# alexpreynolds/starch3

Hardware: AMD Instinct MI355X
Metric: input BED MB/s (cfg2, bzip2 -9, archive bit-identical to CPU starch3 path) (higher is better)
Workload: dtype u8

## Files before the change

### starch_amd/csrc/bz2_bwt3.hip

```cpp
#include "bz2_int.hpp"
#include "bz2_bwt.hpp"

#include <algorithm>
#include <type_traits>

namespace bz {
namespace {

constexpr int PT = 256;
constexpr int PTILE = 32768;
constexpr int PDIG = 12;
constexpr int PNB = 1 << PDIG;
constexpr int PNB_WIDE = 8192;
static_assert(PTILE <= 32768 && PNB_WIDE <= 8192, "k3_scatter_lds packs (digit << 15) | rotation-in-tile");
constexpr int MAXT = (900064 + PTILE - 1) / PTILE;
constexpr uint32_t W_MAX = 64, S1_MAX = 128, S_MAX = 256, M0_MAX = 512, M1_MAX = 1024, M2_MAX = 2048, M3_MAX = 4096;
#ifndef STARCH_L_MIN
#define STARCH_L_MIN 4096
#endif
constexpr uint32_t L_MIN = STARCH_L_MIN;
constexpr uint32_t GB_MIN = 16384;
constexpr uint32_t GB_MAXN = 8192;
constexpr uint32_t HG_MIN_PUSH = 32768;
constexpr uint32_t RBITS = 20;
// ... 1451 lines not shown
            const uint64_t item = shfl64(myitem, gi);
            const uint32_t goff = (uint32_t)__shfl((int)off, (int)gi, 64);
            const uint32_t gstart = valid ? goff : 0u;
            const uint32_t slot = it_slot(item), s = it_start(item), m = it_size(item), par = it_par(item);
            const uint32_t j = valid ? lane - gstart : 0u;
            const uint32_t* sv = (par ? c.scr.V : c.scr.SA) + (uint64_t)slot * c.scr.stride + s;
            const KeySrc ks = key_src(c, slot, par);
            const uint32_t v = sv[j];
            uint32_t ls;
            uint64_t k = elem_key<DBL>(c, ks, slot, s + j, v, ls);
            if (!valid) k = ~0ull;
            uint32_t r = 0;
            if (ng == 1) {
                for (uint32_t q = 0; q < total; ++q) {
                    const uint64_t kq = ((uint64_t)(uint32_t)__builtin_amdgcn_readlane((int)(k >> 32), (int)q) << 32) |
                                        (uint32_t)__builtin_amdgcn_readlane((int)(uint32_t)k, (int)q);
                    r += (kq < k || (kq == k && q < j)) ? 1u : 0u;
                }
            } else {
                const uint32_t maxm = wave_reduce_max(valid ? m : 0u);
                for (uint32_t q = 0; q < maxm; ++q) {
                    const bool in = valid && q < m;
                    const uint64_t kq = shfl64(k, in ? gstart + q : lane);
                    r += (in && (kq < k || (kq == k && q < j))) ? 1u : 0u;
                }
            }
            wave_sync_lds3();
            if (valid) { skey[wid][gstart + r] = k; sval[wid][gstart + r] = v | (ls << 24); }
            wave_sync_lds3();
            const uint64_t key = valid ? skey[wid][lane] : 0;
            const uint32_t val = valid ? sval[wid][lane] : 0;
            const bool head = valid && (j == 0 || skey[wid][lane - 1] != key);
            const bool end = valid && (j + 1 == m || skey[wid][lane + 1] != key);
            const uint32_t hp = wave_incl_scan_max<uint32_t>(head ? lane : 0u) - gstart;
            asm volatile("s_waitcnt vmcnt(0)" ::: "memory");
            uint32_t runs = 0;
            emit_sorted(c, slot, s, j, val & 0xFFFFFFu, valid, hp, end, runs, val >> 24);
            if (c.mode) {
                const uint64_t em = __ballot(end);
                const uint64_t gm = (m >= 64 ? ~0ull : ((1ull << m) - 1ull)) << gstart;
                wave_add_slot(c.L.runs, valid && j == 0, slot, (uint32_t)__popcll(em & gm));
            }
            done += ng;
        }
    }
}

#ifndef STARCH_RANK_UNROLL
#define STARCH_RANK_UNROLL 4
#endif
__device__ __forceinline__ uint32_t rank_in(const uint64_t* xk, uint32_t rs, uint32_t re, uint64_t kj)
{
    uint32_t r = 0;
    uint32_t q = rs;
    if constexpr (STARCH_RANK_UNROLL >= 8) {
        for (; q + 8 <= re; q += 8) {
            uint64_t x[8];
#pragma unroll
            for (int i = 0; i < 8; ++i) x[i] = xk[q + i];
#pragma unroll
            for (int i = 0; i < 8; ++i) r += x[i] < kj ? 1u : 0u;
        }
    }
    if constexpr (STARCH_RANK_UNROLL != 0) {
        for (; q + 4 <= re; q += 4) {
            const uint64_t a = xk[q], b = xk[q + 1], c2 = xk[q + 2], d = xk[q + 3];
            r += (a < kj ? 1u : 0u) + (b < kj ? 1u : 0u) + (c2 < kj ? 1u : 0u) + (d < kj ? 1u : 0u);
        }
    }
    for (; q < re; ++q) r += xk[q] < kj ? 1u : 0u;
    return r;
}

template <int NW>
__device__ __forceinline__ void gsync()
{
    if constexpr (NW == 1) wave_sync_lds3();
    else __syncthreads();
}

template <int E>
struct GrpIn {
    uint64_t item;
    KeySrc ks;
    uint32_t v[E];
    uint32_t v0;
    uint64_t kx[E];
    uint32_t ls[E];
    uint64_t k0;
    uint64_t kb[E];
    uint32_t lb[E];
    uint64_t k0b;
    bool one;
};

template <int NW, int E>
__device__ __forceinline__ void grp_load_vals(const Ctx& c, GrpIn<E>& x, bool ok, int wid, int lane)
{
    if (!ok) x.item = mk_item(0, 0, 1, 0, 0);
    const uint32_t slot = it_slot(x.item), s = it_start(x.item), m = it_size(x.item), par = it_par(x.item);
    const uint32_t* sv = (par ? c.scr.V : c.scr.SA) + (uint64_t)slot * c.scr.stride + s;
    x.ks = key_src(c, slot, par);
#pragma unroll
    for (int e = 0; e < E; ++e) {
        const uint32_t i = (uint32_t)(wid * 64 * E + e * 64 + lane);
        x.v[e] = sv[i < m ? i : 0u];
    }
    x.v0 = sv[0];
}

__device__ __forceinline__ uint32_t pss_rr(const KeySrc& ks, uint32_t r)
{
    const uint32_t rr = r + ks.off;
    return rr >= ks.n ? rr - ks.n : rr;
}
__device__ __forceinline__ uint32_t pss_pr(const KeySrc& ks, uint32_t r) { return r ? r - 1u : ks.n - 1u; }

template <int NW, bool DBL>
constexpr bool defer_keys() { return !DBL && NW == 1; }

template <int NW, int E, bool DBL>
__device__ __forceinline__ void grp_load_keys(const Ctx& c, GrpIn<E>& x, int wid, int lane)
{
    const uint32_t s = it_start(x.item), m = it_size(x.item), slot = it_slot(x.item);
    if constexpr (!defer_keys<NW, DBL>()) {
#pragma unroll
        for (int e = 0; e < E; ++e) {
            const uint32_t i = (uint32_t)(wid * 64 * E + e * 64 + lane);
            x.kx[e] = elem_key<DBL>(c, x.ks, slot, s + (i < m ? i : 0u), x.v[e], x.ls[e]);
        }
        x.k0 = elem_key<DBL>(x.ks, s, x.v0);
    } else {
        const uint64_t* __restrict__ w = x.ks.pss;
        const uint32_t* __restrict__ w32 = reinterpret_cast<const uint32_t*>(w);
        const uint32_t B = x.ks.B;
        x.one = x.ks.off == 0 && (B == 1 || B == 2 || B == 4 || B == 5 || B == 6 || B == 8);
        if (x.one) {
#pragma unroll
            for (int e = 0; e < E; ++e) {
                const uint32_t r = x.v[e];
                const uint64_t q = ((uint64_t)(r ? r - 1u : 0u) * B) >> 6;
                const uint4 kv = *reinterpret_cast<const uint4*>(w + q);
                x.kx[e] = ((uint64_t)kv.y << 32) | kv.x;
                x.kb[e] = ((uint64_t)kv.w << 32) | kv.z;
                if (r == 0) {
                    const uint64_t j = ((uint64_t)(x.ks.n - 1u) * B) >> 5;
                    x.ls[e] = w32[j ^ 1u];
                    x.lb[e] = w32[(j + 1u) ^ 1u];
                }
            }
        } else {
#pragma unroll
            for (int e = 0; e < E; ++e) {
                const uint64_t q = ((uint64_t)pss_rr(x.ks, x.v[e]) * B) >> 6;
                x.kx[e] = w[q];
                x.kb[e] = w[q + 1];
                const uint64_t j = ((uint64_t)pss_pr(x.ks, x.v[e]) * B) >> 5;
                x.ls[e] = w32[j ^ 1u];
                x.lb[e] = w32[(j + 1u) ^ 1u];
            }
        }
        const uint64_t q0 = ((uint64_t)pss_rr(x.ks, x.v0) * x.ks.B) >> 6;
        x.k0 = w[q0];
        x.k0b = w[q0 + 1];
    }
}

template <int NW, int E, bool DBL>
__device__ __forceinline__ void grp_finish_keys(GrpIn<E>& x)
{
    if constexpr (defer_keys<NW, DBL>()) {
        const KeySrc& ks = x.ks;
        if (x.one) {
            const uint32_t B = ks.B;
#pragma unroll
            for (int e = 0; e < E; ++e) {
                const uint32_t r = x.v[e];
                const uint64_t A = x.kx[e], W = x.kb[e];
                if (r) {
                    const uint32_t p0 = (uint32_t)(((uint64_t)(r - 1u) * B) & 63u), pk = p0 + B;
                    x.ls[e] = (uint32_t)(((A << p0) | ((W >> 1) >> (63u - p0))) >> (64u - B));
                    const uint64_t win = pk >= 64u ? (W << (pk - 64u)) : ((A << pk) | ((W >> 1) >> (63u - pk)));
                    x.kx[e] = win >> (64u - ks.kbits);
                } else {
                    x.kx[e] = A >> (64u - ks.kbits);
                    const uint32_t pl = (uint32_t)(((uint64_t)(ks.n - 1u) * B) & 31u);
                    const uint64_t lw = ((uint64_t)x.ls[e] << 32) | x.lb[e];
                    x.ls[e] = (uint32_t)((lw << pl) >> (64u - B));
                }
            }
        } else {
#pragma unroll
        for (int e = 0; e < E; ++e) {
            const uint32_t p = (uint32_t)(((uint64_t)pss_rr(ks, x.v[e]) * ks.B) & 63u);
            const uint64_t v = (x.kx[e] << p) | ((x.kb[e] >> 1) >> (63u - p));
            x.kx[e] = v >> (64u - ks.kbits);
            const uint32_t pl = (uint32_t)(((uint64_t)pss_pr(ks, x.v[e]) * ks.B) & 31u);
            const uint64_t lw = ((uint64_t)x.ls[e] << 32) | x.lb[e];
            x.ls[e] = (uint32_t)((lw << pl) >> (64u - ks.B));
        }
        }
        const uint32_t p0 = (uint32_t)(((uint64_t)pss_rr(ks, x.v0) * ks.B) & 63u);
        const uint64_t v0 = (x.k0 << p0) | ((x.k0b >> 1) >> (63u - p0));
        x.k0 = v0 >> (64u - ks.kbits);
    }
}

#ifndef STARCH_WPE_GRP
#define STARCH_WPE_GRP 1
#endif
#ifndef STARCH_WPE_M2
#define STARCH_WPE_M2 3
#endif
#ifndef STARCH_WPE_S
#define STARCH_WPE_S STARCH_WPE_GRP
#endif
#ifndef STARCH_WPE_M1
#define STARCH_WPE_M1 1
#endif
#ifndef STARCH_WPE_M0
#define STARCH_WPE_M0 6
#endif
constexpr int sort_wpe(int NW, int E)
{
    return NW == 4 && E == 8   ? STARCH_WPE_M2
           : NW == 4 && E == 4 ? STARCH_WPE_M1
           : NW == 4 && E == 2 ? STARCH_WPE_M0
           : (NW == 1 ? (E == 2 ? STARCH_WPE_S : STARCH_WPE_GRP) : 1);
}

template <int NW, int E, bool DBL>
__global__ void __launch_bounds__(NW > 4 ? 64 * NW : 256) __attribute__((amdgpu_waves_per_eu(sort_wpe(NW, E))))
k3_sort_lds(Ctx c, const uint64_t* __restrict__ items,
                                                    const uint32_t* __restrict__ hard_n)
{
    constexpr int IPW = NW >= 4 ? 1 : 4 / NW;
    constexpr int NWV = IPW * NW;
    constexpr int CAP = NW * 64 * E;
    constexpr int IDXB = CAP <= 256 ? 8 : 12;
    constexpr int KEYB = 64 - IDXB;
    constexpr uint64_t KMASK = (1ull << KEYB) - 1ull;
    constexpr int DPT = NW >= 4 ? 1 : 256 / (64 * NW);
    static_assert(CAP <= (1 << IDXB), "index does not fit");
#ifndef STARCH_M2_DB
#define STARCH_M2_DB 11
#endif
    constexpr int DB = CAP <= 128 ? 7 : (CAP <= 256 ? 8 : (CAP <= 1024 ? 10 : (CAP == 2048 ? STARCH_M2_DB : 11)));
    constexpr int NBIN = 1 << DB;
    constexpr int T = NW * 64;
    constexpr int BPT = NBIN / T;
#ifndef STARCH_LIM_NUM
#define STARCH_LIM_NUM 256
#endif
#ifndef STARCH_LIM2_NUM
#define STARCH_LIM2_NUM 512
#endif
    constexpr uint32_t LIMIT = STARCH_LIM_NUM / E;
    __shared__ uint64_t xk_all[IPW][CAP];
    __shared__ uint32_t vb_all[IPW][CAP];
    __shared__ uint16_t bst_all[IPW][NBIN + 2];
    constexpr int UR = NBIN > 256 * NW ? NBIN : 256 * NW;
    __shared__ uint32_t ur_all[IPW][UR];
    __shared__ uint32_t sc_all[IPW][NW + 1];
    constexpr int NB2 = NW == 1 ? 256 : 1024;
    constexpr uint32_t LIMIT2 = STARCH_LIM2_NUM / E;
    __shared__ uint32_t c2_all[IPW][NB2 + 1];
    __shared__ uint32_t sc2_all[IPW][NW + 1];
    __shared__ uint64_t red_all[NWV];
    __shared__ uint32_t wmax_all[NWV];
    __shared__ uint32_t flag_all[NWV];
    __shared__ uint32_t tc_all[NW + 1 > 5 ? NW + 1 : 5];
    uint32_t tacc = 0;
    const int tid = threadIdx.x, lane = tid & 63, wave = tid >> 6;
    const int g = wave / NW, wid = wave % NW, w0 = g * NW;
    uint64_t* xk = xk_all[g];
    uint32_t* wcnt = ur_all[g] + wid * 256;
    uint32_t* sc = sc_all[g];
    const uint64_t lt = lanemask_lt();
    constexpr uint32_t NONE = 0xFFFFFFFFu;
    const uint32_t nwk = gridDim.x * (uint32_t)IPW;
    const uint32_t e_end = hard_n ? *hard_n : 0u;
    uint32_t it_s = blockIdx.x * (uint32_t)IPW + (uint32_t)g;
    const uint32_t xs8 = blockIdx.x & 7u;
    const uint32_t s_end = hard_n ? e_end : c.qseg[xs8 + 1];
    const uint32_t s_nwk = hard_n ? nwk : (gridDim.x >> 3) * (uint32_t)IPW;
    if (!hard_n) it_s = c.qseg[xs8] + (blockIdx.x >> 3) * (uint32_t)IPW + (uint32_t)g;
    auto next_item = [&]() -> uint32_t {
        const uint32_t r = it_s < s_end ? it_s : NONE;
        it_s += s_nwk;
        return r;
    };
    uint32_t it = next_item();
    uint32_t it1 = it != NONE ? next_item() : NONE;
    GrpIn<E> cur, nxt;
    cur.item = it != NONE ? items[it] : 0ull;
    grp_load_vals<NW, E>(c, cur, it != NONE, wid, lane);
    grp_load_keys<NW, E, DBL>(c, cur, wid, lane);
    nxt.item = it1 != NONE ? items[it1] : 0ull;
    grp_load_vals<NW, E>(c, nxt, it1 != NONE, wid, lane);
    while (it != NONE) {
    const uint64_t item = cur.item;
    const uint32_t slot = it_slot(item), s = it_start(item), m = it_size(item);
    grp_finish_keys<NW, E, DBL>(cur);
    gsync<NW>();

    uint64_t k[E];
    uint64_t diff = 0;
#pragma unroll
    for (int e = 0; e < E; ++e) {
        const uint32_t i = (uint32_t)(wid * 64 * E + e * 64 + lane);
        if (i < m) {
            diff |= cur.kx[e] ^ cur.k0;
            k[e] = ((cur.kx[e] & KMASK) << IDXB) | i;
            vb_all[g][i] = cur.v[e] | (cur.ls[e] << 24);
        } else {
            k[e] = ~0ull;
        }
    }
    grp_load_keys<NW, E, DBL>(c, nxt, wid, lane);
    diff = wave_reduce_or64(diff);
    if constexpr (NW > 1) {
        if (lane == 0) red_all[wave] = diff;
        __syncthreads();
        diff = 0;
#pragma unroll
        for (int w = 0; w < NW; ++w) diff |= red_all[w0 + w];
    }
    if ((diff >> KEYB) && tid % (64 * NW) == 0) atomicOr(&c.L.ctr[C_ERR], 1u);

    bool moved = false;
    const uint64_t kdiff = diff & KMASK;
    if (kdiff) {
        uint16_t* bst = bst_all[g];
        uint32_t* bcur = ur_all[g];
        const int tg = wid * 64 + lane;
        const int hb = 63 - __clzll((long long)kdiff);
        const int lo = hb + 1 - DB > 0 ? hb + 1 - DB : 0;
        for (int q = tg; q < NBIN; q += T) bcur[q] = 0;
        gsync<NW>();
        uint32_t dg[E];
#pragma unroll
        for (int e = 0; e < E; ++e) {
            dg[e] = (uint32_t)((k[e] >> (lo + IDXB)) & (uint64_t)(NBIN - 1));
            if ((uint32_t)(wid * 64 * E + e * 64 + lane) < m) atomicAdd(&bcur[dg[e]], 1u);
        }
        gsync<NW>();
        uint32_t loc[BPT], sum = 0, mx = 0;
#pragma unroll
        for (int q = 0; q < BPT; ++q) {
            loc[q] = bcur[tg * BPT + q];
            sum += loc[q];
            mx = loc[q] > mx ? loc[q] : mx;
        }
        const uint32_t incl = wave_incl_scan_add(sum);
        uint32_t run = incl - sum;
        mx = wave_reduce_max(mx);
        if constexpr (NW > 1) {
            if (lane == 63) sc[wid] = incl;
            if (lane == 0) wmax_all[wave] = mx;
            __syncthreads();
            for (int w = 0; w < wid; ++w) run += sc[w];
            mx = 0;
            for (int w = 0; w < NW; ++w) mx = wmax_all[w0 + w] > mx ? wmax_all[w0 + w] : mx;
        }
        auto rank_place = [&](auto&& range_of) {
            uint32_t p[E];
#pragma unroll
            for (int e = 0; e < E; ++e) {
                const uint32_t j = (uint32_t)(wid * 64 * E + e * 64 + lane);
                p[e] = j;
                if (j < m) {
                    const uint64_t kj = xk[j];
                    uint32_t rs, re;
                    range_of(kj, rs, re);
                    p[e] = rs + rank_in(xk, rs, re, kj);
                    k[e] = kj;
                }
            }
            gsync<NW>();
#pragma unroll
            for (int e = 0; e < E; ++e) xk[p[e]] = k[e];
            gsync<NW>();
#pragma unroll
            for (int e = 0; e < E; ++e) k[e] = xk[wid * 64 * E + e * 64 + lane];
        };
        if (mx <= LIMIT) {
#pragma unroll
            for (int q = 0; q < BPT; ++q) { bst[tg * BPT + q] = run; bcur[tg * BPT + q] = run; run += loc[q]; }
            if (tg == T - 1) bst[NBIN] = run;
            gsync<NW>();
#pragma unroll
            for (int e = 0; e < E; ++e)
                if ((uint32_t)(wid * 64 * E + e * 64 + lane) < m) xk[atomicAdd(&bcur[dg[e]], 1u)] = k[e];
            gsync<NW>();
            rank_place([&](uint64_t kj, uint32_t& rs, uint32_t& re) {
                const uint32_t d = (uint32_t)((kj >> (lo + IDXB)) & (uint64_t)(NBIN - 1));
                rs = bst[d];
                re = bst[d + 1];
            });
            moved = true;
        } else if (lo > 0) {
            uint32_t* c2 = c2_all[g];
            uint32_t* sc2 = sc2_all[g];
            uint32_t nbl = 0;
#pragma unroll
            for (int q = 0; q < BPT; ++q) nbl += loc[q] > LIMIT ? 1u : 0u;
            const uint32_t binc = wave_incl_scan_add(nbl);
            uint32_t bb = binc - nbl, nbig = 0;
            if constexpr (NW > 1) {
                if (lane == 63) sc2[wid] = binc;
                __syncthreads();
                for (int w = 0; w < NW; ++w) { if (w < wid) bb += sc2[w]; nbig += sc2[w]; }
            } else {
                nbig = (uint32_t)__builtin_amdgcn_readlane((int)binc, 63);
            }
            uint32_t w2 = 0;
#ifndef STARCH_W2_MAX
#define STARCH_W2_MAX 6
#endif
            while (w2 < STARCH_W2_MAX && (nbig << (w2 + 1)) <= (uint32_t)NB2) ++w2;
            if (w2 > (uint32_t)lo) w2 = (uint32_t)lo;
            const int lo2 = lo - (int)w2;
            const uint32_t nb2 = nbig << w2;
#pragma unroll
            for (int q = 0; q < BPT; ++q) {
                bst[tg * BPT + q] = run;
                bcur[tg * BPT + q] = loc[q] > LIMIT ? (0x80000000u | ((bb++) << w2)) : run;
                run += loc[q];
            }
            if (tg == T - 1) bst[NBIN] = run;
            for (uint32_t q = (uint32_t)tg; q < nb2; q += T) c2[q] = 0;
            gsync<NW>();
            uint32_t b2[E];
#pragma unroll
            for (int e = 0; e < E; ++e) {
                b2[e] = ~0u;
                if ((uint32_t)(wid * 64 * E + e * 64 + lane) < m) {
                    const uint32_t x = bcur[dg[e]];
                    if (x >> 31) {
                        b2[e] = (x & 0x7FFFFFFFu) + (uint32_t)((k[e] >> (lo2 + IDXB)) & ((1ull << w2) - 1ull));
                        atomicAdd(&c2[b2[e]], 1u);
                    }
                }
            }
            gsync<NW>();
            constexpr int BPT2 = (NB2 + T - 1) / T;
            uint32_t l2[BPT2], s2 = 0, m2 = 0;
#pragma unroll
            for (int q = 0; q < BPT2; ++q) {
                const uint32_t ix = (uint32_t)(tg * BPT2 + q);
                l2[q] = ix < nb2 ? c2[ix] : 0u;
                s2 += l2[q];
                m2 = l2[q] > m2 ? l2[q] : m2;
            }
            const uint32_t inc2 = wave_incl_scan_add(s2);
            uint32_t r2 = inc2 - s2;
            m2 = wave_reduce_max(m2);
            if constexpr (NW > 1) {
                __syncthreads();
                if (lane == 63) sc2[wid] = inc2;
                if (lane == 0) wmax_all[wave] = m2;
                __syncthreads();
                for (int w = 0; w < wid; ++w) r2 += sc2[w];
                for (int w = 0; w < NW; ++w) m2 = wmax_all[w0 + w] > m2 ? wmax_all[w0 + w] : m2;
            }
#pragma unroll
            for (int q = 0; q < BPT2; ++q) {
                const uint32_t ix = (uint32_t)(tg * BPT2 + q);
                if (ix < nb2) c2[ix] = r2;
                r2 += l2[q];
            }
            gsync<NW>();
            if (m2 <= LIMIT2) {
                uint32_t sb[E];
#pragma unroll
                for (int e = 0; e < E; ++e) sb[e] = b2[e] != ~0u ? c2[bcur[dg[e]] & 0x7FFFFFFFu] : 0u;
                gsync<NW>();
#pragma unroll
                for (int e = 0; e < E; ++e) {
                    if ((uint32_t)(wid * 64 * E + e * 64 + lane) < m) {
                        const uint32_t p = b2[e] != ~0u ? bst[dg[e]] + atomicAdd(&c2[b2[e]], 1u) - sb[e]
                                                        : atomicAdd(&bcur[dg[e]], 1u);
                        xk[p] = k[e];
                    }
                }
                gsync<NW>();
                rank_place([&](uint64_t kj, uint32_t& rs, uint32_t& re) {
                    const uint32_t d = (uint32_t)((kj >> (lo + IDXB)) & (uint64_t)(NBIN - 1));
                    const uint32_t x = bcur[d];
                    if (x >> 31) {
                        const uint32_t base = x & 0x7FFFFFFFu;
                        const uint32_t b = base + (uint32_t)((kj >> (lo2 + IDXB)) & ((1ull << w2) - 1ull));
                        const uint32_t s0 = base ? c2[base - 1] : 0u;
                        rs = bst[d] + (b ? c2[b - 1] : 0u) - s0;
                        re = bst[d] + c2[b] - s0;
                    } else {
                        rs = bst[d];
                        re = bst[d + 1];
                    }
                });
                moved = true;
            }
        } else {
            gsync<NW>();
        }
    }
    bool lsd_moved = false;
    for (int dbit = 0; dbit < KEYB && !moved; dbit += 8) {
        if ((kdiff >> dbit & 0xffull) == 0) continue;
        for (int q = lane; q < 256; q += 64) wcnt[q] = 0;
        wave_sync_lds3();
        uint32_t dg[E], rk[E], ld[E], ret[E];
#pragma unroll
        for (int e = 0; e < E; ++e) {
            const uint32_t d = (uint32_t)((k[e] >> (dbit + IDXB)) & 255u);
            uint64_t peers = ~0ull;
#pragma unroll
            for (int bb = 0; bb < 8; ++bb) {
                const uint64_t bal = __ballot((d >> bb) & 1u);
                peers &= ((d >> bb) & 1u) ? bal : ~bal;
            }
            const uint32_t leader = (uint32_t)__ffsll((unsigned long long)peers) - 1u;
            dg[e] = d;
            ld[e] = leader;
            rk[e] = (uint32_t)__popcll(peers & lt);
            ret[e] = 0;
            if ((uint32_t)lane == leader) ret[e] = atomicAdd(&wcnt[d], (uint32_t)__popcll(peers));
        }
#pragma unroll
        for (int e = 0; e < E; ++e) rk[e] += (uint32_t)__shfl((int)ret[e], (int)ld[e], 64);
        gsync<NW>();
        {
            const int t = wid * 64 + lane;
            const bool has = t * DPT < 256;
            uint32_t loc[DPT], sum = 0;
#pragma unroll
            for (int q = 0; q < DPT; ++q) {
                uint32_t a = 0;
#pragma unroll
                for (int w = 0; w < NW; ++w) a += has ? ur_all[g][w * 256 + t * DPT + q] : 0u;
                loc[q] = a;
                sum += a;
            }
            const uint32_t incl = wave_incl_scan_add(sum);
            uint32_t run = incl - sum;
            if constexpr (NW > 1) {
                if (lane == 63) sc[wid] = incl;
                __syncthreads();
                for (int w = 0; w < wid; ++w) run += sc[w];
            }
#pragma unroll
            for (int q = 0; q < DPT && has; ++q) {
                uint32_t r = run;
#pragma unroll
                for (int w = 0; w < NW; ++w) {
                    const uint32_t xx = ur_all[g][w * 256 + t * DPT + q];
                    ur_all[g][w * 256 + t * DPT + q] = r;
                    r += xx;
                }
                run += loc[q];
            }
        }
        gsync<NW>();
#pragma unroll
        for (int e = 0; e < E; ++e) xk[rk[e] + wcnt[dg[e]]] = k[e];
        gsync<NW>();
#pragma unroll
        for (int e = 0; e < E; ++e) k[e] = xk[wid * 64 * E + e * 64 + lane];
        lsd_moved = true;
    }
    moved |= lsd_moved;
    if (!moved) {
#pragma unroll
        for (int e = 0; e < E; ++e) xk[wid * 64 * E + e * 64 + lane] = k[e];
    }
    gsync<NW>();
    bool tie_here = false;
#pragma unroll
    for (int e = 0; e < E; ++e) {
        const uint32_t j = (uint32_t)(wid * 64 * E + e * 64 + lane);
        if (j > 0 && j < m && ((xk[j - 1] ^ k[e]) >> IDXB) == 0) tie_here = true;
    }
    bool ties = __ballot(tie_here) != 0;
    if constexpr (NW > 1) {
        if (lane == 0) flag_all[wave] = ties ? 1u : 0u;
        __syncthreads();
        ties = false;
        for (int w = 0; w < NW; ++w) ties |= flag_all[w0 + w] != 0;
    }
    uint32_t hp[E];
    if (!ties) {
#pragma unroll
        for (int e = 0; e < E; ++e) hp[e] = (uint32_t)(wid * 64 * E + e * 64 + lane);
    } else {
        uint32_t carry = 0;
#pragma unroll
        for (int e = 0; e < E; ++e) {
            const uint32_t j = (uint32_t)(wid * 64 * E + e * 64 + lane);
            const bool head = j < m && (j == 0 || ((xk[j - 1] ^ k[e]) >> IDXB) != 0);
            uint32_t xx = wave_incl_scan_max<uint32_t>(head ? j : 0u);
            xx = xx > carry ? xx : carry;
            hp[e] = xx;
            carry = (uint32_t)__builtin_amdgcn_readlane((int)xx, 63);
        }
        if constexpr (NW > 1) {
            if (lane == 0) wmax_all[wave] = carry;
            __syncthreads();
            uint32_t pre = 0;
            for (int w = 0; w < wid; ++w) pre = wmax_all[w0 + w] > pre ? wmax_all[w0 + w] : pre;
#pragma unroll
            for (int e = 0; e < E; ++e) hp[e] = hp[e] > pre ? hp[e] : pre;
        }
    }
    uint32_t runs = 0, tcnt = 0;
    uint64_t tm[E];
#pragma unroll
    for (int e = 0; e < E; ++e) {
        const uint32_t j = (uint32_t)(wid * 64 * E + e * 64 + lane);
        const bool valid = j < m;
        const uint32_t vb = valid ? vb_all[g][(uint32_t)(k[e] & ((1u << IDXB) - 1u))] : 0u;
        const bool end = valid && (!ties || j + 1 == m || ((xk[j + 1] ^ k[e]) >> IDXB) != 0);
        emit_vals(c, slot, s, j, vb & 0xFFFFFFu, valid, hp[e], vb >> 24);
        const bool tie = end && j > hp[e];
        tm[e] = __ballot(tie);
        tcnt += (uint32_t)__popcll(tm[e]);
        tacc += tie ? j - hp[e] + 1u : 0u;
        runs += (uint32_t)__popcll(__ballot(end));
    }
    if (c.mode && lane == 0 && runs) atomicAdd(&c.L.runs[slot], runs);
    if (ties) {
        uint32_t tb = tie_reserve<NW>(c, tcnt, tc_all, wid, lane);
        uint64_t* tl = c.L.t[c.tsel];
#pragma unroll
        for (int e = 0; e < E; ++e) {
            const uint32_t j = (uint32_t)(wid * 64 * E + e * 64 + lane);
            if ((tm[e] >> lane) & 1ull) tl[tb + (uint32_t)__popcll(tm[e] & lt)] = mk_item(slot, s + hp[e], j - hp[e] + 1u, 0, 0);
            tb += (uint32_t)__popcll(tm[e]);
        }
    }
    const uint32_t it2 = it1 != NONE ? next_item() : NONE;
    cur = nxt;
    nxt.item = it2 != NONE ? items[it2] : 0ull;
    grp_load_vals<NW, E>(c, nxt, it2 != NONE, wid, lane);
    it = it1;
    it1 = it2;
    }
    tacc = wave_reduce_add<uint32_t>(tacc);
    if (lane == 0 && tacc) atomicAdd(c.L.ctr + C_TS0 + c.tsel, tacc);
}

#ifndef STARCH_HARD_Q
#define STARCH_HARD_Q 32
#endif
constexpr uint32_t HARD_Q = STARCH_HARD_Q;

template <int NW, int E, bool DBL>
__global__ void __launch_bounds__(256) __attribute__((amdgpu_waves_per_eu(sort_wpe(NW, E))))
k3_sort_grp(Ctx c, const uint64_t* __restrict__ items,
                                                    uint64_t* __restrict__ hard)
{
    constexpr int IPW = 4 / NW;
    constexpr int CAP = NW * 64 * E;
    constexpr int IDXB = CAP <= 256 ? 8 : 12;
    constexpr int KEYB = 64 - IDXB;
    constexpr uint64_t KMASK = (1ull << KEYB) - 1ull;
    static_assert(CAP <= (1 << IDXB), "index does not fit");
    constexpr int DB = CAP <= 128 ? 7 : (CAP <= 256 ? 8 : (CAP <= 1024 ? 10 : 11));
    constexpr int NBIN = 1 << DB;
    constexpr int T = NW * 64;
    constexpr int BPT = NBIN / T;
    __shared__ uint64_t xk_all[IPW][CAP];
    __shared__ uint32_t vb_all[IPW][CAP];
    __shared__ uint32_t bst_all[IPW][NBIN + 1];
    __shared__ uint32_t bcur_all[IPW][NBIN];
    __shared__ uint32_t sc_all[IPW][NW + 1];
    __shared__ uint64_t red_all[4];
    __shared__ uint32_t wsq_all[4];
    __shared__ uint32_t wmax_all[4];
    __shared__ uint32_t flag_all[4];
    __shared__ uint32_t tc_all[5];
    uint32_t tacc = 0;
    const uint64_t lt = lanemask_lt();
    const int tid = threadIdx.x, lane = tid & 63, wave = tid >> 6;
    const int g = wave / NW, wid = wave % NW, w0 = g * NW;
    uint64_t* xk = xk_all[g];
    uint32_t* sc = sc_all[g];
    uint32_t* bst = bst_all[g];
    uint32_t* bcur = bcur_all[g];
    const int tg = wid * 64 + lane;
#ifndef STARCH_GRP_CHUNK
#define STARCH_GRP_CHUNK 32
#endif
    static_assert(NW == 1, "k3_sort_grp: one wave per group");
    __shared__ uint32_t qs[8];
    const uint32_t xs = xcc_id();
    load_qsizes_binned(c, qs);
#ifndef STARCH_GRP_CHUNK_S2
#define STARCH_GRP_CHUNK_S2 16
#endif
    WaveQueue<E == 4 ? STARCH_GRP_CHUNK_S2 : STARCH_GRP_CHUNK> wq;
    constexpr uint32_t NONE = 0xFFFFFFFFu;
    uint32_t it = wq.next(c.qhead, qs, c.qseg, xs);
    uint32_t it1 = it != NONE ? wq.next(c.qhead, qs, c.qseg, xs) : NONE;
    uint32_t it2 = it1 != NONE ? wq.next(c.qhead, qs, c.qseg, xs) : NONE;
    GrpIn<E> cur, nxt;
    cur.item = it != NONE ? items[it] : 0ull;
    nxt.item = it1 != NONE ? items[it1] : 0ull;
    grp_load_vals<NW, E>(c, cur, it != NONE, wid, lane);
    grp_load_keys<NW, E, DBL>(c, cur, wid, lane);
    grp_load_vals<NW, E>(c, nxt, it1 != NONE, wid, lane);
    uint64_t nitem2 = it2 != NONE ? items[it2] : 0ull;
    while (it != NONE) {
    const uint64_t item = cur.item;
    const uint32_t slot = it_slot(item), s = it_start(item), m = it_size(item);
    grp_finish_keys<NW, E, DBL>(cur);
    gsync<NW>();

    uint64_t k[E];
    uint64_t diff = 0;
#pragma unroll
    for (int e = 0; e < E; ++e) {
        const uint32_t i = (uint32_t)(wid * 64 * E + e * 64 + lane);
        if (i < m) {
            diff |= cur.kx[e] ^ cur.k0;
            k[e] = ((cur.kx[e] & KMASK) << IDXB) | i;
            vb_all[g][i] = cur.v[e] | (cur.ls[e] << 24);
        } else {
            k[e] = ~0ull;
        }
    }
    grp_load_keys<NW, E, DBL>(c, nxt, wid, lane);
    diff = wave_reduce_or64(diff);
    if constexpr (NW > 1) {
        if (lane == 0) red_all[wave] = diff;
        __syncthreads();
        diff = 0;
#pragma unroll
        for (int w = 0; w < NW; ++w) diff |= red_all[w0 + w];
    }
    if ((diff >> KEYB) && tg == 0) atomicOr(&c.L.ctr[C_ERR], 1u);

    bool is_hard = false;
    const uint64_t kdiff = diff & KMASK;
    if (kdiff) {
        const int hb = 63 - __clzll((long long)kdiff);
        const int lo = hb + 1 - DB > 0 ? hb + 1 - DB : 0;
        for (int q = tg; q < NBIN; q += T) bcur[q] = 0;
        gsync<NW>();
        uint32_t dg[E];
#pragma unroll
        for (int e = 0; e < E; ++e) {
            dg[e] = (uint32_t)((k[e] >> (lo + IDXB)) & (uint64_t)(NBIN - 1));
            if ((uint32_t)(wid * 64 * E + e * 64 + lane) < m) atomicAdd(&bcur[dg[e]], 1u);
        }
        gsync<NW>();
        uint32_t loc[BPT], sum = 0, sq = 0;
#pragma unroll
        for (int q = 0; q < BPT; ++q) {
            loc[q] = bcur[tg * BPT + q];
            sum += loc[q];
            sq += loc[q] * loc[q];
        }
        const uint32_t incl = wave_incl_scan_add(sum);
        uint32_t run = incl - sum;
        sq = wave_reduce_add(sq);
        if constexpr (NW > 1) {
            if (lane == 63) sc[wid] = incl;
            if (lane == 0) wsq_all[wave] = sq;
            __syncthreads();
            for (int w = 0; w < wid; ++w) run += sc[w];
            sq = 0;
            for (int w = 0; w < NW; ++w) sq += wsq_all[w0 + w];
        }
        is_hard = sq > HARD_Q * m;
        if (!is_hard) {
#pragma unroll
            for (int q = 0; q < BPT; ++q) { bst[tg * BPT + q] = run; bcur[tg * BPT + q] = run; run += loc[q]; }
            if (tg == T - 1) bst[NBIN] = run;
            gsync<NW>();
#pragma unroll
            for (int e = 0; e < E; ++e)
                if ((uint32_t)(wid * 64 * E + e * 64 + lane) < m) xk[atomicAdd(&bcur[dg[e]], 1u)] = k[e];
            gsync<NW>();
            uint32_t pos[E];
#pragma unroll
            for (int e = 0; e < E; ++e) {
                const uint32_t j = (uint32_t)(wid * 64 * E + e * 64 + lane);
                pos[e] = j;
                if (j < m) {
                    const uint64_t kj = xk[j];
                    const uint32_t d = (uint32_t)((kj >> (lo + IDXB)) & (uint64_t)(NBIN - 1));
                    const uint32_t bs = bst[d], be = bst[d + 1];
                    pos[e] = bs + rank_in(xk, bs, be, kj);
                    k[e] = kj;
                }
            }
            gsync<NW>();
#pragma unroll
            for (int e = 0; e < E; ++e) xk[pos[e]] = k[e];
        } else {
            gsync<NW>();
            if (tg == 0) hard[atomicAdd(&c.L.ctr[C_H], 1u)] = item;
        }
    } else {
#pragma unroll
        for (int e = 0; e < E; ++e) xk[wid * 64 * E + e * 64 + lane] = k[e];
    }
    const uint32_t it3 = it2 != NONE ? wq.next(c.qhead, qs, c.qseg, xs) : NONE;
    const uint64_t nitem3 = it3 != NONE ? items[it3] : 0ull;
    if (!is_hard) {
    gsync<NW>();
#pragma unroll
    for (int e = 0; e < E; ++e) k[e] = xk[wid * 64 * E + e * 64 + lane];
    bool tie_here = false;
#pragma unroll
    for (int e = 0; e < E; ++e) {
        const uint32_t j = (uint32_t)(wid * 64 * E + e * 64 + lane);
        if (j > 0 && j < m && ((xk[j - 1] ^ k[e]) >> IDXB) == 0) tie_here = true;
    }
    bool ties = __ballot(tie_here) != 0;
    if constexpr (NW > 1) {
        if (lane == 0) flag_all[wave] = ties ? 1u : 0u;
        __syncthreads();
        ties = false;
        for (int w = 0; w < NW; ++w) ties |= flag_all[w0 + w] != 0;
    }
    uint32_t hp[E];
    if (!ties) {
#pragma unroll
        for (int e = 0; e < E; ++e) hp[e] = (uint32_t)(wid * 64 * E + e * 64 + lane);
    } else {
        uint32_t carry = 0;
#pragma unroll
        for (int e = 0; e < E; ++e) {
            const uint32_t j = (uint32_t)(wid * 64 * E + e * 64 + lane);
            const bool head = j < m && (j == 0 || ((xk[j - 1] ^ k[e]) >> IDXB) != 0);
            uint32_t xx = wave_incl_scan_max<uint32_t>(head ? j : 0u);
            xx = xx > carry ? xx : carry;
            hp[e] = xx;
            carry = (uint32_t)__builtin_amdgcn_readlane((int)xx, 63);
        }
        if constexpr (NW > 1) {
            if (lane == 0) wmax_all[wave] = carry;
            __syncthreads();
            uint32_t pre = 0;
            for (int w = 0; w < wid; ++w) pre = wmax_all[w0 + w] > pre ? wmax_all[w0 + w] : pre;
#pragma unroll
            for (int e = 0; e < E; ++e) hp[e] = hp[e] > pre ? hp[e] : pre;
        }
    }
    uint32_t runs = 0, tcnt = 0;
    uint64_t tm[E];
#pragma unroll
    for (int e = 0; e < E; ++e) {
        const uint32_t j = (uint32_t)(wid * 64 * E + e * 64 + lane);
        const bool valid = j < m;
        const uint32_t vb = valid ? vb_all[g][(uint32_t)(k[e] & ((1u << IDXB) - 1u))] : 0u;
        const bool end = valid && (!ties || j + 1 == m || ((xk[j + 1] ^ k[e]) >> IDXB) != 0);
        emit_vals(c, slot, s, j, vb & 0xFFFFFFu, valid, hp[e], vb >> 24);
        const bool tie = end && j > hp[e];
        tm[e] = __ballot(tie);
        tcnt += (uint32_t)__popcll(tm[e]);
        tacc += tie ? j - hp[e] + 1u : 0u;
        runs += (uint32_t)__popcll(__ballot(end));
    }
    if (c.mode && lane == 0 && runs) atomicAdd(&c.L.runs[slot], runs);
    if (ties) {
        uint32_t tb = tie_reserve<NW>(c, tcnt, tc_all, wid, lane);
        uint64_t* tl = c.L.t[c.tsel];
#pragma unroll
        for (int e = 0; e < E; ++e) {
            const uint32_t j = (uint32_t)(wid * 64 * E + e * 64 + lane);
            if ((tm[e] >> lane) & 1ull) tl[tb + (uint32_t)__popcll(tm[e] & lt)] = mk_item(slot, s + hp[e], j - hp[e] + 1u, 0, 0);
            tb += (uint32_t)__popcll(tm[e]);
        }
    }
    }
    cur = nxt;
    nxt.item = nitem2;
    nitem2 = nitem3;
    grp_load_vals<NW, E>(c, nxt, it2 != NONE, wid, lane);
    it = it1;
    it1 = it2;
    it2 = it3;
    }
    tacc = wave_reduce_add<uint32_t>(tacc);
    if (lane == 0 && tacc) atomicAdd(c.L.ctr + C_TS0 + c.tsel, tacc);
}

constexpr uint32_t CT_IPT = 16;

__global__ void __launch_bounds__(256) k3_classify_text(Ctx c, const uint64_t* __restrict__ items, uint32_t nitems)
{
    __shared__ uint32_t cls_cnt[8], cls_base[8];
    const uint32_t tid = threadIdx.x, lane = tid & 63;
    if (tid < 8) cls_cnt[tid] = 0;
    __syncthreads();
    const uint64_t i0 = (uint64_t)blockIdx.x * 256u * CT_IPT + tid;
    uint64_t it[CT_IPT];
    uint32_t cnt[8] = {0, 0, 0, 0, 0, 0, 0, 0}, tied = 0;
#pragma unroll
    for (uint32_t k = 0; k < CT_IPT; ++k) {
        const uint64_t i = i0 + (uint64_t)k * 256u;
        it[k] = i < nitems ? items[i] : 0ull;
        if (i < nitems) {
            const uint32_t m = it_size(it[k]);
            ++cnt[size_class(m)];
            tied += m;
        }
    }
    uint32_t off[8];
#pragma unroll
// ... 544 lines not shown
```

Baseline: 85780.

## Cut group barriers in bucket sort by merging reductions and reusing atomic offsets

Removes several workgroup barriers from the per-item group sort in the BWT kernel. The bin-clear and diff-reduction now share one barrier. The histogram atomics return each element's offset within its bin, so the scatter pass needs no second round of atomics. Cross-wave prefix sums are built from ballots and atomics during the histogram, and the tie flag and head-carry exchange are merged into a single barrier. This packs offsets into the upper bits of the digit registers, which assumes bins and offsets fit in 16 bits. It also changes how the c2 and bst range arithmetic is computed, so any mistake would break bit-identical output.

```diff
diff --git a/starch_amd/csrc/bz2_bwt3.hip b/starch_amd/csrc/bz2_bwt3.hip
--- a/starch_amd/csrc/bz2_bwt3.hip
+++ b/starch_amd/csrc/bz2_bwt3.hip
@@ -1777,7 +1777,6 @@
     const uint64_t item = cur.item;
     const uint32_t slot = it_slot(item), s = it_start(item), m = it_size(item);
     grp_finish_keys<NW, E, DBL>(cur);
-    gsync<NW>();
 
     uint64_t k[E];
     uint64_t diff = 0;
@@ -1787,16 +1786,26 @@
         if (i < m) {
             diff |= cur.kx[e] ^ cur.k0;
             k[e] = ((cur.kx[e] & KMASK) << IDXB) | i;
-            vb_all[g][i] = cur.v[e] | (cur.ls[e] << 24);
         } else {
             k[e] = ~0ull;
         }
     }
+    diff = wave_reduce_or64(diff);
+    uint32_t* bcur = ur_all[g];
+    const int tg = wid * 64 + lane;
+    for (int q = tg; q < NBIN; q += T) bcur[q] = 0;
+    if constexpr (NW > 1) {
+        if (tg < NW) sc[tg] = 0;
+        if (lane == 0) red_all[wave] = diff;
+    }
+    gsync<NW>();
+#pragma unroll
+    for (int e = 0; e < E; ++e) {
+        const uint32_t i = (uint32_t)(wid * 64 * E + e * 64 + lane);
+        if (i < m) vb_all[g][i] = cur.v[e] | (cur.ls[e] << 24);
+    }
     grp_load_keys<NW, E, DBL>(c, nxt, wid, lane);
-    diff = wave_reduce_or64(diff);
     if constexpr (NW > 1) {
-        if (lane == 0) red_all[wave] = diff;
-        __syncthreads();
         diff = 0;
 #pragma unroll
         for (int w = 0; w < NW; ++w) diff |= red_all[w0 + w];
@@ -1807,35 +1816,46 @@
     const uint64_t kdiff = diff & KMASK;
     if (kdiff) {
         uint16_t* bst = bst_all[g];
-        uint32_t* bcur = ur_all[g];
-        const int tg = wid * 64 + lane;
         const int hb = 63 - __clzll((long long)kdiff);
         const int lo = hb + 1 - DB > 0 ? hb + 1 - DB : 0;
-        for (int q = tg; q < NBIN; q += T) bcur[q] = 0;
+        constexpr int BW = 64 * BPT;
+        uint32_t dg[E], mx = 0;
+        uint32_t below[NW] = {};
+#pragma unroll
+        for (int e = 0; e < E; ++e) {
+            const bool valid = (uint32_t)(wid * 64 * E + e * 64 + lane) < m;
+            dg[e] = (uint32_t)((k[e] >> (lo + IDXB)) & (uint64_t)(NBIN - 1));
+            if constexpr (NW > 1) {
+                const uint32_t dv = valid ? dg[e] : (uint32_t)NBIN;
+#pragma unroll
+                for (int w = 1; w < NW; ++w) below[w] += (uint32_t)__popcll(__ballot(dv < (uint32_t)(w * BW)));
+            }
+            if (valid) {
+                const uint32_t off = atomicAdd(&bcur[dg[e]], 1u);
+                mx = off + 1u > mx ? off + 1u : mx;
+                dg[e] |= off << 16;
+            }
+        }
+        mx = wave_reduce_max(mx);
+        if constexpr (NW > 1) {
+            uint32_t mine = 0;
+#pragma unroll
+            for (int w = 1; w < NW; ++w) mine = lane == w ? below[w] : mine;
+            if (lane >= 1 && lane < NW && mine) atomicAdd(&sc[lane], mine);
+            if (lane == 0) wmax_all[wave] = mx;
+        }
         gsync<NW>();
-        uint32_t dg[E];
-#pragma unroll
-        for (int e = 0; e < E; ++e) {
-            dg[e] = (uint32_t)((k[e] >> (lo + IDXB)) & (uint64_t)(NBIN - 1));
-            if ((uint32_t)(wid * 64 * E + e * 64 + lane) < m) atomicAdd(&bcur[dg[e]], 1u);
-        }
-        gsync<NW>();
-        uint32_t loc[BPT], sum = 0, mx = 0;
+        uint32_t loc[BPT], sum = 0;
 #pragma unroll
         for (int q = 0; q < BPT; ++q) {
             loc[q] = bcur[tg * BPT + q];
             sum += loc[q];
-            mx = loc[q] > mx ? loc[q] : mx;
-        }
-        const uint32_t incl = wave_incl_scan_add(sum);
-        uint32_t run = incl - sum;
-        mx = wave_reduce_max(mx);
+        }
+        uint32_t run = wave_incl_scan_add(sum) - sum;
         if constexpr (NW > 1) {
-            if (lane == 63) sc[wid] = incl;
-            if (lane == 0) wmax_all[wave] = mx;
-            __syncthreads();
-            for (int w = 0; w < wid; ++w) run += sc[w];
+            run += sc[wid];
             mx = 0;
+#pragma unroll
             for (int w = 0; w < NW; ++w) mx = wmax_all[w0 + w] > mx ? wmax_all[w0 + w] : mx;
         }
         auto rank_place = [&](auto&& range_of) {
@@ -1861,12 +1881,12 @@
         };
         if (mx <= LIMIT) {
 #pragma unroll
-            for (int q = 0; q < BPT; ++q) { bst[tg * BPT + q] = run; bcur[tg * BPT + q] = run; run += loc[q]; }
+            for (int q = 0; q < BPT; ++q) { bst[tg * BPT + q] = run; run += loc[q]; }
             if (tg == T - 1) bst[NBIN] = run;
             gsync<NW>();
 #pragma unroll
             for (int e = 0; e < E; ++e)
-                if ((uint32_t)(wid * 64 * E + e * 64 + lane) < m) xk[atomicAdd(&bcur[dg[e]], 1u)] = k[e];
+                if ((uint32_t)(wid * 64 * E + e * 64 + lane) < m) xk[bst[dg[e] & 0xFFFFu] + (dg[e] >> 16)] = k[e];
             gsync<NW>();
             rank_place([&](uint64_t kj, uint32_t& rs, uint32_t& re) {
                 const uint32_t d = (uint32_t)((kj >> (lo + IDXB)) & (uint64_t)(NBIN - 1));
@@ -1900,7 +1920,7 @@
 #pragma unroll
             for (int q = 0; q < BPT; ++q) {
                 bst[tg * BPT + q] = run;
-                bcur[tg * BPT + q] = loc[q] > LIMIT ? (0x80000000u | ((bb++) << w2)) : run;
+                bcur[tg * BPT + q] = loc[q] > LIMIT ? (0x80000000u | ((bb++) << w2)) : 0u;
                 run += loc[q];
             }
             if (tg == T - 1) bst[NBIN] = run;
@@ -1911,10 +1931,10 @@
             for (int e = 0; e < E; ++e) {
                 b2[e] = ~0u;
                 if ((uint32_t)(wid * 64 * E + e * 64 + lane) < m) {
-                    const uint32_t x = bcur[dg[e]];
+                    const uint32_t x = bcur[dg[e] & 0xFFFFu];
                     if (x >> 31) {
-                        b2[e] = (x & 0x7FFFFFFFu) + (uint32_t)((k[e] >> (lo2 + IDXB)) & ((1ull << w2) - 1ull));
-                        atomicAdd(&c2[b2[e]], 1u);
+                        const uint32_t b = (x & 0x7FFFFFFFu) + (uint32_t)((k[e] >> (lo2 + IDXB)) & ((1ull << w2) - 1ull));
+                        b2[e] = b | (atomicAdd(&c2[b], 1u) << 16);
                     }
                 }
             }
@@ -1945,17 +1965,20 @@
                 if (ix < nb2) c2[ix] = r2;
                 r2 += l2[q];
             }
+            if (tg == T - 1) c2[nb2] = r2;
             gsync<NW>();
             if (m2 <= LIMIT2) {
-                uint32_t sb[E];
-#pragma unroll
-                for (int e = 0; e < E; ++e) sb[e] = b2[e] != ~0u ? c2[bcur[dg[e]] & 0x7FFFFFFFu] : 0u;
-                gsync<NW>();
 #pragma unroll
                 for (int e = 0; e < E; ++e) {
                     if ((uint32_t)(wid * 64 * E + e * 64 + lane) < m) {
-                        const uint32_t p = b2[e] != ~0u ? bst[dg[e]] + atomicAdd(&c2[b2[e]], 1u) - sb[e]
-                                                        : atomicAdd(&bcur[dg[e]], 1u);
+                        uint32_t p = bst[dg[e] & 0xFFFFu];
+                        if (b2[e] != ~0u) {
+                            const uint32_t b = b2[e] & 0xFFFFu;
+                            const uint32_t base = b - (uint32_t)((k[e] >> (lo2 + IDXB)) & ((1ull << w2) - 1ull));
+                            p += c2[b] - c2[base] + (b2[e] >> 16);
+                        } else {
+                            p += dg[e] >> 16;
+                        }
                         xk[p] = k[e];
                     }
                 }
@@ -1966,9 +1989,9 @@
                     if (x >> 31) {
                         const uint32_t base = x & 0x7FFFFFFFu;
                         const uint32_t b = base + (uint32_t)((kj >> (lo2 + IDXB)) & ((1ull << w2) - 1ull));
-                        const uint32_t s0 = base ? c2[base - 1] : 0u;
-                        rs = bst[d] + (b ? c2[b - 1] : 0u) - s0;
-                        re = bst[d] + c2[b] - s0;
+                        const uint32_t s0 = bst[d] - c2[base];
+                        rs = s0 + c2[b];
+                        re = s0 + c2[b + 1];
                     } else {
                         rs = bst[d];
                         re = bst[d + 1];
@@ -2048,27 +2071,24 @@
     if (!moved) {
 #pragma unroll
         for (int e = 0; e < E; ++e) xk[wid * 64 * E + e * 64 + lane] = k[e];
-    }
-    gsync<NW>();
+        gsync<NW>();
+    }
     bool tie_here = false;
 #pragma unroll
     for (int e = 0; e < E; ++e) {
         const uint32_t j = (uint32_t)(wid * 64 * E + e * 64 + lane);
         if (j > 0 && j < m && ((xk[j - 1] ^ k[e]) >> IDXB) == 0) tie_here = true;
     }
-    bool ties = __ballot(tie_here) != 0;
-    if constexpr (NW > 1) {
-        if (lane == 0) flag_all[wave] = ties ? 1u : 0u;
-        __syncthreads();
-        ties = false;
-        for (int w = 0; w < NW; ++w) ties |= flag_all[w0 + w] != 0;
-    }
+    const bool wties = __ballot(tie_here) != 0;
+    bool ties = wties;
     uint32_t hp[E];
-    if (!ties) {
+    uint32_t carry = 0;
+    if (!wties) {
 #pragma unroll
         for (int e = 0; e < E; ++e) hp[e] = (uint32_t)(wid * 64 * E + e * 64 + lane);
+        const uint32_t wend = (uint32_t)((wid + 1) * 64 * E);
+        carry = m > (uint32_t)(wid * 64 * E) ? (m < wend ? m : wend) - 1u : 0u;
     } else {
-        uint32_t carry = 0;
 #pragma unroll
         for (int e = 0; e < E; ++e) {
             const uint32_t j = (uint32_t)(wid * 64 * E + e * 64 + lane);
@@ -2078,11 +2098,19 @@
             hp[e] = xx;
             carry = (uint32_t)__builtin_amdgcn_readlane((int)xx, 63);
         }
-        if constexpr (NW > 1) {
-            if (lane == 0) wmax_all[wave] = carry;
-            __syncthreads();
-            uint32_t pre = 0;
-            for (int w = 0; w < wid; ++w) pre = wmax_all[w0 + w] > pre ? wmax_all[w0 + w] : pre;
+    }
+    if constexpr (NW > 1) {
+        if (lane == 0) flag_all[wave] = carry | (wties ? 0x80000000u : 0u);
+        __syncthreads();
+        uint32_t pre = 0, any = 0;
+#pragma unroll
+        for (int w = 0; w < NW; ++w) {
+            const uint32_t x = flag_all[w0 + w];
+            any |= x;
+            if (w < wid) pre = (x & 0x7FFFFFFFu) > pre ? (x & 0x7FFFFFFFu) : pre;
+        }
+        ties = (any >> 31) != 0;
+        if (wties) {
 #pragma unroll
             for (int e = 0; e < E; ++e) hp[e] = hp[e] > pre ? hp[e] : pre;
         }
```

After: 86590 (median of 6 runs). About the same (+0.9%).
